# Bioinfo-Tools/PANGEA-plus

Hardware: AMD Instinct MI355X
Metric: classified reads/sec (+ HBM GB/s fraction), 150 bp vs 1 Gbp db, 1/2/4/8 GPU (higher is better)
Workload: dtype u64 (2-bit packed bases, integer scores)

## Files before the change

pangea-plus_amd/csrc/classify.hip:

```cpp
#include <algorithm>
#include <chrono>

#include "bitops.hpp"
#include "consensus_core.hpp"
#include "engine.hpp"

namespace pgx {

struct Diag {
	const uint64_t *rw, *ra;
	const uint64_t *dbw, *dba;
	int64_t dstart;
	int lo, hi;
};

template <bool AMB> __device__ __forceinline__ uint64_t mmw(const Diag &D, int w)
{
	int b0 = 32 * w;
	if (b0 + 32 <= D.lo || b0 >= D.hi)
		return kEven;
	uint64_t x = D.rw[w] ^ window64(D.dbw, D.dstart + b0);
	uint64_t m = (x | (x >> 1)) & kEven;
	if (AMB) {
		if (D.ra)
			m |= D.ra[w];
		if (D.dba)
			m |= window64(D.dba, D.dstart + b0);
	}
	m |= kEven & ~spaced_range(D.lo - b0, D.hi - b0);
	return m;
}

__device__ __forceinline__ uint64_t compress_even(uint64_t x)
{
	x = (x | (x >> 1)) & 0x3333333333333333ull;
	x = (x | (x >> 2)) & 0x0F0F0F0F0F0F0F0Full;
	x = (x | (x >> 4)) & 0x00FF00FF00FF00FFull;
	x = (x | (x >> 8)) & 0x0000FFFF0000FFFFull;
	x = (x | (x >> 16)) & 0x00000000FFFFFFFFull;
	return x;
}

template <bool AMB, int NW> struct DenseMask {
	static constexpr bool kHasWindows = true;
	static constexpr int kBits = 64 * NW;
	uint64_t m[NW];
	int lo, hi;
	__device__ __forceinline__ static uint64_t pick(const uint64_t (&a)[NW], int wi)
	{
		uint64_t v = 0;
#pragma unroll
		for (int k = 0; k < NW; k++)
			v = wi == k ? a[k] : v;
		return v;
	}
	__device__ __forceinline__ static uint64_t below(int n) { return n <= 0 ? 0ull : (n >= 64 ? ~0ull : ((1ull << n) - 1)); }
	__device__ __forceinline__ static uint64_t from(int n) { return n <= 0 ? ~0ull : (n >= 64 ? 0ull : (~0ull << n)); }
	__device__ __forceinline__ void build(const Diag &D)
	{
		lo = D.lo;
		hi = D.hi;
		const int64_t wi = D.dstart >> 5;
		const int sh = (int)(D.dstart & 31) * 2;
		uint64_t dbv[2 * NW + 1], rwv[2 * NW];
#pragma unroll
		for (int w = 0; w < 2 * NW + 1; w++)
			dbv[w] = D.dbw[wi + w];
#pragma unroll
		for (int w = 0; w < 2 * NW; w++)
			rwv[w] = D.rw[w];
		uint64_t d[2 * NW];
#pragma unroll
		for (int w = 0; w < 2 * NW; w++) {
			const uint64_t win = sh ? (dbv[w] >> sh) | (dbv[w + 1] << (64 - sh)) : dbv[w];
			const uint64_t x = rwv[w] ^ win;
			uint64_t mm = (x | (x >> 1)) & kEven;
			if (AMB) {
				if (D.ra)
					mm |= D.ra[w];
				if (D.dba)
					mm |= window64(D.dba, D.dstart + 32 * w);
			}
			d[w] = compress_even(mm);
		}
#pragma unroll
		for (int k = 0; k < NW; k++)
			m[k] = (d[2 * k] | (d[2 * k + 1] << 32)) | below(lo - 64 * k) | from(hi - 64 * k);
	}
	struct Win {
		uint64_t w[NW];
	};
	template <int K> __device__ __forceinline__ static void and_shr(const uint64_t (&a)[NW], const uint64_t (&src)[NW], uint64_t (&o)[NW])
	{
#pragma unroll
		for (int k = 0; k < NW; k++) {
			const uint64_t up = k + 1 < NW ? src[k + 1] : 0ull;
			o[k] = a[k] & ((src[k] >> K) | (up << (64 - K)));
		}
	}
	__device__ __forceinline__ Win seed_windows() const
	{
		uint64_t r[NW], a2[NW], a4[NW], a8[NW], b16[NW], c24[NW];
#pragma unroll
		for (int k = 0; k < NW; k++)
			r[k] = ~m[k];
		and_shr<1>(r, r, a2);
		and_shr<2>(a2, a2, a4);
		and_shr<4>(a4, a4, a8);
		and_shr<8>(a8, a8, b16);
		and_shr<16>(b16, a8, c24);
		Win w;
		and_shr<24>(c24, a4, w.w);
		return w;
	}
	__device__ __forceinline__ static bool win_any_below(const Win &w, int n)
	{
		uint64_t any = 0;
#pragma unroll
		for (int k = 0; k < NW; k++)
			any |= w.w[k] & below(n - 64 * k);
		return any != 0;
	}
	__device__ __forceinline__ static int first_set_ge(const uint64_t (&a)[NW], int n)
	{
		int r = kBits;
#pragma unroll
		for (int k = NW - 1; k >= 0; k--) {
			const uint64_t v = a[k] & from(n - 64 * k);
			r = v ? 64 * k + __ffsll((unsigned long long)v) - 1 : r;
		}
		return r;
	}
	__device__ __forceinline__ static int win_first_ge(const Win &w, int n) { return first_set_ge(w.w, n); }
	__device__ __forceinline__ bool flagged(int p) const { return (pick(m, p >> 6) >> (p & 63)) & 1ull; }
	__device__ __forceinline__ int count_range(int a, int b) const
	{
		a = a > lo ? a : lo;
		b = b < hi ? b : hi;
		int c = 0;
#pragma unroll
		for (int k = 0; k < NW; k++)
			c += __popcll(m[k] & from(a - 64 * k) & below(b - 64 * k));
		return c;
	}
	__device__ __forceinline__ int first_ge(int pos) const
	{
		if (pos >= hi)
			return hi;
		const int r = first_set_ge(m, pos);
		return r < hi ? r : hi;
	}
	__device__ __forceinline__ int last_lt(int pos) const
	{
		if (pos <= lo)
			return lo - 1;
		int r = -1;
#pragma unroll
		for (int k = 0; k < NW; k++) {
			const uint64_t v = m[k] & below(pos - 64 * k);
			r = v ? 64 * k + 63 - __clzll((long long)v) : r;
		}
		return r >= lo ? r : lo - 1;
	}
	struct Fwd {
		uint64_t w;
		int wi;
	};
	__device__ __forceinline__ Fwd fwd_from(int k) const
	{
		const int pos = k + 1;
		Fwd c;
		c.wi = pos >> 6;
		c.w = pick(m, c.wi) & (~0ull << (pos & 63));
		return c;
	}
	__device__ __forceinline__ int fwd_next(Fwd &c) const
	{
		while (!c.w) {
			c.wi++;
			if (c.wi >= NW)
				return hi;
			c.w = pick(m, c.wi);
		}
		const int r = c.wi * 64 + __ffsll((unsigned long long)c.w) - 1;
		c.w &= c.w - 1;
		return r < hi ? r : hi;
	}
	struct Bwd {
		uint64_t w;
		int wi;
	};
	__device__ __forceinline__ Bwd bwd_from(int k) const
	{
		Bwd c;
		if (k <= 0) {
			c.w = 0;
			c.wi = 0;
			return c;
		}
		const int q = k - 1, bb = q & 63;
		c.wi = q >> 6;
		c.w = pick(m, c.wi) & (bb == 63 ? ~0ull : ((2ull << bb) - 1));
		return c;
	}
	__device__ __forceinline__ int bwd_next(Bwd &c) const
	{
		while (!c.w) {
			if (c.wi == 0)
				return lo - 1;
			c.wi--;
			c.w = pick(m, c.wi);
		}
		const int bb = 63 - __clzll((long long)c.w);
		c.w ^= 1ull << bb;
		const int r = c.wi * 64 + bb;
		return r >= lo ? r : lo - 1;
	}
};

template <bool AMB> struct LazyMask {
	static constexpr bool kHasWindows = false;
	struct Win {
	};
	Diag D;
	int lo, hi;
	__device__ __forceinline__ void build(const Diag &d)
	{
		D = d;
		lo = d.lo;
		hi = d.hi;
	}
	__device__ __forceinline__ int count_range(int, int) const { return 15; }
	__device__ __forceinline__ bool flagged(int p) const { return first_ge(p) == p; }
	__device__ __forceinline__ int first_ge(int pos) const
	{
		if (pos >= hi)
			return hi;
		int w = pos >> 5;
		uint64_t m = mmw<AMB>(D, w) & ~((1ull << (2 * (pos & 31))) - 1);
		while (!m) {
			w++;
			if (32 * w >= hi)
				return hi;
			m = mmw<AMB>(D, w);
		}
		int r = 32 * w + ((__ffsll((unsigned long long)m) - 1) >> 1);
		return r < hi ? r : hi;
	}
	__device__ __forceinline__ int last_lt(int pos) const
	{
		if (pos <= lo)
			return lo - 1;
		int q = pos - 1, w = q >> 5, bit = q & 31;
		uint64_t keep = bit == 31 ? ~0ull : ((1ull << (2 * bit + 2)) - 1);
		uint64_t m = mmw<AMB>(D, w) & keep;
		while (!m) {
			if (32 * w <= lo)
				return lo - 1;
			w--;
			m = mmw<AMB>(D, w);
		}
		int r = 32 * w + ((63 - __clzll((long long)m)) >> 1);
		return r >= lo ? r : lo - 1;
	}
	struct Fwd {
		int k;
	};
	__device__ __forceinline__ Fwd fwd_from(int k) const { return Fwd{ k }; }
	__device__ __forceinline__ int fwd_next(Fwd &c) const { return c.k = first_ge(c.k + 1); }
	struct Bwd {
		int k;
	};
	__device__ __forceinline__ Bwd bwd_from(int k) const { return Bwd{ k }; }
	__device__ __forceinline__ int bwd_next(Bwd &c) const { return c.k = last_lt(c.k); }
};

constexpr int kStage = 128;
constexpr int kDeal = 2;
constexpr int kQueue = 64 * (kDeal + 1);
constexpr int kWavesPerBlock = 4;

typedef uint32_t u32x4 __attribute__((ext_vector_type(4)));
union HitWords {
	pgx_hit h;
	u32x4 v[2];
};
__device__ __forceinline__ void store_hit_stream(pgx_hit *p, const pgx_hit &h)
{
	HitWords w;
	w.h = h;
	u32x4 *d = reinterpret_cast<u32x4 *>(p);
	__builtin_nontemporal_store(w.v[0], d);
	__builtin_nontemporal_store(w.v[1], d + 1);
}


constexpr int kDiagSlots = 128;
constexpr int kDiagProbes = 8;
constexpr uint32_t kNoDiag = 0xFFFFFFFFu;

struct WaveLds {
	union {
		pgx_hit hit[kStage];
		uint4 chit[2 * kStage];
	};
	uint32_t qp[kQueue], qmeta[kQueue], qsubj[kQueue], qs0[kQueue], qs1[kQueue];
	uint32_t diag[2][2][kDiagSlots / 2];
	uint64_t uwin[2][2][8];
	unsigned int n[2];
	unsigned int direct[2];
};

struct OutView {
	pgx_hit *main, *ovf;
	uint8_t *main_key, *ovf_key;
	uint8_t *main_reg;
	int reg_shift;
	unsigned long long main_cap, ovf_cap;
	unsigned long long *counters;
};
constexpr unsigned int kChunk = 2048;

__device__ __forceinline__ uint4 pack_hit(const pgx_hit &h)
{
	const uint32_t minus = h.sstart > h.send;
	return make_uint4((uint32_t)h.subject, (uint32_t)h.sstart, (uint32_t)h.qstart | ((uint32_t)h.qend << 16) | (minus << 31),
			  (uint32_t)h.score | ((uint32_t)h.mismatch << 16) | ((uint32_t)h.gapopen << 24));
}

__device__ __forceinline__ pgx_hit unpack_hit(const uint4 c, uint32_t read)
{
	pgx_hit h;
	h.read = (int32_t)read;
	h.subject = (int32_t)c.x;
	h.sstart = (int32_t)c.y;
	h.qstart = (int32_t)(c.z & 0xFFFFu);
	h.qend = (int32_t)((c.z >> 16) & 0x7FFFu);
	const int span = h.qend - h.qstart;
	h.send = (c.z >> 31) ? h.sstart - span : h.sstart + span;
	h.score = (int32_t)(c.w & 0xFFFFu);
	h.mismatch = (uint16_t)((c.w >> 16) & 0xFFu);
	h.gapopen = (uint16_t)(c.w >> 24);
	return h;
}

__device__ __forceinline__ uint4 pack_seed(const pgx_hit &h)
{
	const uint32_t sd = (uint32_t)h.send;
	return make_uint4((uint32_t)h.subject, (uint32_t)h.sstart, (uint32_t)h.qend | (((sd >> 1) & 0x7FFu) << 15) | (sd << 31),
			  (uint32_t)h.mismatch | ((uint32_t)h.gapopen << 4) | ((sd >> 12) << 8));
}

__device__ __forceinline__ pgx_hit unpack_seed(const uint4 c, uint32_t read, uint32_t woff, int L)
{
	pgx_hit h;
	h.read = (int32_t)read;
	h.subject = (int32_t)c.x;
	h.qstart = (int32_t)woff;
	h.qend = (int32_t)(c.z & 0x7FFFu);
	h.sstart = (int32_t)c.y;
	h.send = (int32_t)((c.z >> 31) | (((c.z >> 15) & 0x7FFu) << 1) | ((c.w >> 8) << 12));
	h.score = L;
	h.mismatch = (uint16_t)(c.w & 15u);
	h.gapopen = (uint16_t)((c.w >> 4) & 15u);
	return h;
}

__device__ __forceinline__ uint8_t seed_key(const pgx_hit &h) { return (uint8_t)((h.mismatch & 15u) | ((h.gapopen & 15u) << 4)); }

template <bool PACKED>
__device__ __forceinline__ void emit_hit(WaveLds *st, int rs, const OutView &ov, const pgx_hit &h, bool gapped)
{
	unsigned int slot = atomicAdd(&st->n[rs], 1u);
	if (slot < (unsigned)kStage) {
		if (PACKED)
			st->chit[rs * kStage + slot] = gapped ? pack_seed(h) : pack_hit(h);
		else
			st->hit[slot] = h;
	} else {
		atomicAdd(&st->direct[rs], 1u);
		unsigned long long g = atomicAdd(&ov.counters[4], 1ull);
		if (g < ov.ovf_cap) {
			ov.ovf[g] = h;
			if (gapped)
				ov.ovf_key[g] = seed_key(h);
		}
	}
}

__device__ __forceinline__ bool uwin_any(const uint64_t *uw, int a, int b)
{
	if (b < a)
		return false;
	for (int w = a >> 6; w <= (b >> 6); w++) {
		uint64_t v = uw[w];
		if (w == (a >> 6))
			v &= ~0ull << (a & 63);
		if (w == (b >> 6) && (b & 63) != 63)
			v &= (2ull << (b & 63)) - 1ull;
		if (v)
			return true;
	}
	return false;
}

template <bool AMB, class Mask, class Emit>
__device__ __forceinline__ void process_candidate(const DbView &db, const uint64_t *rw, const uint64_t *ra, const uint64_t *uw, int L,
						   uint32_t read, uint32_t woff, int strand, int qp, uint32_t p, bool tested, bool claimed, uint32_t s,
						   uint32_t s_start, uint32_t s_end, Emit &emit, unsigned long long &n_runs)
{
	if (p + (uint32_t)kSeedK > s_end)
		return;
	Diag D;
	D.rw = rw;
	D.ra = ra;
	D.dbw = db.words;
	D.dba = db.amb;

	D.dstart = (int64_t)p - qp;
	if (AMB && db.amb && db.amb_blk) {
		const int64_t a = D.dstart > 0 ? D.dstart : 0, b = D.dstart + L - 1;
		uint32_t any = 0;
		for (int64_t blk = a >> kBlkShift; blk <= (b >> kBlkShift); blk++)
			any |= (db.amb_blk[blk >> 5] >> (blk & 31)) & 1u;
		if (!any)
			D.dba = nullptr;
	}
	int64_t lo64 = (int64_t)s_start - D.dstart, hi64 = (int64_t)s_end - D.dstart;
	D.lo = lo64 > 0 ? (int)lo64 : 0;
	D.hi = hi64 < L ? (int)hi64 : L;
	Mask M;
	M.build(D);
	if (PGX_DBG_STOP(db) == 4) {
		n_runs += (unsigned long long)(M.first_ge(qp) & 1);
		return;
	}

	int pos, run_start = 0;
	typename Mask::Win W;
	bool whole = false;
	if constexpr (Mask::kHasWindows)
		whole = claimed;
	if (whole) {
		if constexpr (Mask::kHasWindows) {
			W = M.seed_windows();
			if (uw) {
#pragma unroll
				for (int k = 0; k < Mask::kBits / 64; k++)
					W.w[k] &= uw[k];
			}
			run_start = Mask::win_first_ge(W, 0);
		}
		if (run_start >= D.hi)
			return;
		if (uw)
			run_start = M.last_lt(run_start) + 1;
		n_runs++;
		if (PGX_DBG_STOP(db) == 5 || PGX_DBG_STOP(db) == 6)
			return;
	} else {
		const int lm = M.last_lt(qp);
		if (!tested && qp >= kProbeStride && lm < qp - kProbeStride)
			return;
		const int re = M.first_ge(qp);
		if (re < qp + kSeedK)
			return;
		run_start = lm + 1;
		if (re - run_start < kWord)
			return;
		if constexpr (Mask::kHasWindows) {
			W = M.seed_windows();
			if (uw) {
#pragma unroll
				for (int k = 0; k < Mask::kBits / 64; k++)
					W.w[k] &= uw[k];
				if (Mask::win_first_ge(W, run_start) > re - kWord)
					return;
			}
			n_runs++;
			if (PGX_DBG_STOP(db) == 5)
				return;
			if (Mask::win_any_below(W, run_start))
				return;
		} else {
			if (uw && !uwin_any(uw, run_start, re - kWord))
				return;
			n_runs++;
			if (PGX_DBG_STOP(db) == 5)
				return;
			pos = D.lo;
			while (pos < run_start) {
				int m1 = M.first_ge(pos);
				if (m1 - pos >= kWord && (!uw || uwin_any(uw, pos, m1 - kWord)))
					return;
				pos = m1 + 1;
			}
		}
		if (PGX_DBG_STOP(db) == 6)
			return;
	}
	int covered = D.lo;
	pos = run_start;
	while (pos < D.hi) {
		const int e = M.first_ge(pos);
		const int len = e - pos;
		bool seeds = len >= kWord && pos >= covered;
		if constexpr (!Mask::kHasWindows)
			seeds = seeds && (!uw || uwin_any(uw, pos, e - kWord));
		if (seeds) {
			int best = 0, cur = 0, bl = pos, nmm = 0, mm_best = 0;
			int k = pos - 1;
			typename Mask::Bwd cl = M.bwd_from(k);
			while (k >= D.lo) {
				cur -= 2;
				nmm++;
				if (best - cur > kXdrop)
					break;
				const int p2 = M.bwd_next(cl);
				cur += k - 1 - p2;
				const bool up = cur > best;
				best = up ? cur : best;
				bl = up ? p2 + 1 : bl;
				mm_best = up ? nmm : mm_best;
				k = p2;
			}
			int bestr = 0, br = e - 1, mmr_best = 0;
			cur = 0;
			nmm = 0;
			k = e;
			typename Mask::Fwd cr = M.fwd_from(k);
			while (k < D.hi) {
				cur -= 2;
				nmm++;
				if (bestr - cur > kXdrop)
					break;
				const int n2 = M.fwd_next(cr);
				cur += n2 - (k + 1);
				const bool up = cur > bestr;
				bestr = up ? cur : bestr;
				br = up ? n2 - 1 : br;
				mmr_best = up ? nmm : mmr_best;
				k = n2;
			}
			pgx_hit h;
			h.read = (int32_t)read;
			h.subject = (int32_t)s;
			h.score = len + best + bestr;
			h.mismatch = (uint16_t)(mm_best + mmr_best);
			h.gapopen = 0;
			const int64_t sl = D.dstart + bl - (int64_t)s_start + 1, sr = D.dstart + br - (int64_t)s_start + 1;
			if (!strand) {
				h.qstart = bl + 1;
				h.qend = br + 1;
				h.sstart = (int32_t)sl;
				h.send = (int32_t)sr;
			} else {
				h.qstart = L - br;
				h.qend = L - bl;
				h.sstart = (int32_t)sr;
				h.send = (int32_t)sl;
			}
			if (db.gapped) {
				int q = bl + (br - bl) / 2;
				while (M.flagged(q))
					q--;
				int anchor = M.last_lt(q) + 1;
				anchor = anchor > bl ? anchor : bl;
				int b0l = 0, b0r = 0, kl = 14, kr = 14;
				if constexpr (Mask::kHasWindows) {
					const int ml = M.count_range(bl, anchor), mr = (int)h.mismatch - ml;
					b0l = ml <= 18 ? 2 * (anchor - bl) - 6 * ml : 0;
					b0r = mr <= 18 ? 2 * (br + 1 - anchor) - 6 * mr : 0;
					b0l = b0l > 0 && b0l < 2047 ? b0l : 0;
					b0r = b0r > 0 && b0r < 2047 ? b0r : 0;
					kl = (2 * anchor - b0l) / 5;
					kr = (2 * (L - anchor) - b0r) / 5;
					kl = kl < 14 ? kl : 14;
					kr = kr < 14 ? kr : 14;
					if (L > db.deep_from) {
						kl = (ml + (bl > 0 ? 10 : 0)) / 3;
						kr = (mr + (br + 1 < L ? 10 : 0)) / 3;
						kl = kl < 14 ? kl : 14;
						kr = kr < 14 ? kr : 14;
					}
				}
				h.qstart = (int32_t)woff;
				h.qend = anchor;
				h.sstart = (int32_t)(uint32_t)(D.dstart + anchor);
				h.send = strand | (b0l << 1) | (b0r << 12);
				h.score = L;
				h.mismatch = (uint16_t)kl;
				h.gapopen = (uint16_t)kr;
			}
			if (PGX_DBG_STOP(db) != 7)
				emit(h);
			covered = br + 1;
		}
		if constexpr (Mask::kHasWindows) {
			pos = Mask::win_first_ge(W, covered > e ? covered : e + 1);
			if (uw && pos < D.hi)
				pos = M.last_lt(pos) + 1;
		} else
			pos = covered > e + 1 ? covered : e + 1;
	}
}

__device__ __forceinline__ void lds_fence()
{
	asm volatile("s_waitcnt lgkmcnt(0)" ::: "memory");
	__builtin_amdgcn_wave_barrier();
}

template <bool AMB, int NW, bool LISTED, bool DUST>
__global__ __launch_bounds__(64 * kWavesPerBlock, NW == 8 ? 3 : 4) void k_seed_extend(DbView db, ReadsView rd, OutView ov,
								      uint32_t *__restrict__ read_cnt,
								      uint32_t *__restrict__ read_start)
{
	constexpr bool DENSE = NW > 0;
	constexpr int RPW = DENSE ? 2 : 1;
	constexpr int LPR = 64 / RPW;
	constexpr unsigned int SLOT_CAP = kStage;
	__shared__ WaveLds s_lds[kWavesPerBlock];
	const int wave = threadIdx.x >> 6, lane = threadIdx.x & 63;
	const int my_rs = lane / LPR, my_li = lane % LPR;
	WaveLds *st = &s_lds[wave];
	unsigned long long n_probe = 0, n_post = 0, n_runs = 0, n_main = 0, n_surv = 0;
	unsigned long long chunk_base = 0;
	unsigned int chunk_used = kChunk;
	const unsigned long long lt_mask = lane ? (~0ull >> (64 - lane)) : 0ull;

	for (uint32_t rbase = (blockIdx.x * kWavesPerBlock + wave) * RPW; rbase < rd.n; rbase += gridDim.x * kWavesPerBlock * RPW) {
		const bool hasB = RPW == 2 && rbase + 1 < rd.n;
		const uint32_t rA = LISTED ? rd.list[rbase] : rbase, rB = LISTED ? (hasB ? rd.list[rbase + 1] : 0u) : rbase + 1;
		const int LA = (int)rd.len[rA], LB = hasB ? (int)rd.len[rB] : 0;
		const uint32_t wA = rd.woff[rA], wB = hasB ? rd.woff[rB] : 0u;
		const int L = my_rs ? LB : LA;
		const uint32_t w0 = my_rs ? wB : wA;
		const int nps = L >= kSeedK ? (L - kSeedK) / kProbeStride + 1 : 0;
		const int P = 2 * nps;
		const int PA = LA >= kSeedK ? 2 * ((LA - kSeedK) / kProbeStride + 1) : 0;
		const int PB = LB >= kSeedK ? 2 * ((LB - kSeedK) / kProbeStride + 1) : 0;
		const int Pmax = PA > PB ? PA : PB;
		unsigned int emitted[2] = { 0, 0 }, q_n = 0;
		bool frag[2] = { false, false };
		if (lane == 0) {
			st->n[0] = st->n[1] = 0;
			st->direct[0] = st->direct[1] = 0;
		}
		if (RPW == 2) {
#pragma unroll
			for (int k = 0; k < 2 * kDiagSlots / 64; k++)
				(&st->diag[0][0][0])[k * 64 + lane] = kNoDiag;
		}
		const bool dustA = DUST && rd.dustwin_f && rd.dust_any[rA] != 0, dustB = DUST && rd.dustwin_f && hasB && rd.dust_any[rB] != 0;
		if (DUST && DENSE && (dustA || dustB) && lane < 32) {
			const int us = lane >> 4, ustr = (lane >> 3) & 1, uk = lane & 7;
			const int uL = us ? LB : LA;
			uint64_t v = 0;
			if ((us ? dustB : dustA) && uk < (uL + 63) / 64)
				v = (ustr ? rd.dustwin_r : rd.dustwin_f)[(us ? wB : wA) + uk];
			st->uwin[us][ustr][uk] = v;
		}
		lds_fence();

		auto spill = [&](int rs) {
			unsigned int n = st->n[rs];
			if (n > SLOT_CAP)
				n = SLOT_CAP;
			unsigned long long base = 0;
			if (lane == 0)
				base = atomicAdd(&ov.counters[4], (unsigned long long)n);
			base = __shfl(base, 0);
			for (unsigned int i = lane; i < n; i += 64)
				if (base + i < ov.ovf_cap) {
					const pgx_hit hh = RPW == 2 ? (db.gapped ? unpack_seed(st->chit[rs * SLOT_CAP + i], rs ? rB : rA, rs ? wB : wA, rs ? LB : LA)
										  : unpack_hit(st->chit[rs * SLOT_CAP + i], rs ? rB : rA))
								     : st->hit[i];
					ov.ovf[base + i] = hh;
					if (db.gapped)
						ov.ovf_key[base + i] = seed_key(hh);
				}
			if (rs)
				emitted[1] += n, frag[1] = true;
			else
				emitted[0] += n, frag[0] = true;
			lds_fence();
			if (lane == 0)
				st->n[rs] = 0;
			lds_fence();
		};

		auto drain = [&](unsigned int cnt) {
			q_n -= cnt;
			if ((unsigned)lane < cnt && PGX_DBG_STOP(db) != 3) {
				const uint32_t p = st->qp[q_n + lane], meta = st->qmeta[q_n + lane];
				const uint32_t sj = st->qsubj[q_n + lane], s0 = st->qs0[q_n + lane], s1 = st->qs1[q_n + lane];
				const int strand = (int)(meta >> 31), rs = (int)((meta >> 29) & 1), qp = (int)(meta & 0x0FFFFFFFu);
				const bool tested = (meta >> 30) & 1, claimed = (meta >> 28) & 1;
				const uint32_t cw0 = rs ? wB : wA, cr = rs ? rB : rA;
				const int cL = rs ? LB : LA;
				const uint64_t *rw = (strand ? rd.rc : rd.fwd) + cw0;
				const uint64_t *ra = nullptr;
				if (AMB) {
					const uint64_t *a = strand ? rd.rc_amb : rd.fwd_amb;
					ra = a ? a + cw0 : nullptr;
				}
				const uint64_t *uw = nullptr;
				if (DUST && (rs ? dustB : dustA))
					uw = DENSE ? st->uwin[rs][strand] : (strand ? rd.dustwin_r : rd.dustwin_f) + cw0;
				auto emit = [&](const pgx_hit &hh) { emit_hit<RPW == 2>(st, rs, ov, hh, db.gapped != 0); };
				if (DENSE)
					process_candidate<AMB, DenseMask<AMB, (NW > 0 ? NW : 3)>>(db, rw, ra, uw, cL, cr, cw0, strand, qp, p, tested, claimed, sj, s0, s1, emit, n_runs);
				else
					process_candidate<AMB, LazyMask<AMB>>(db, rw, ra, uw, cL, cr, cw0, strand, qp, p, tested, claimed, sj, s0, s1, emit, n_runs);
			}
			lds_fence();
			if (st->n[0] > SLOT_CAP / 2)
				spill(0);
			if (RPW == 2 && st->n[1] > SLOT_CAP / 2)
				spill(1);
		};

		for (int pbase = 0; pbase < Pmax; pbase += LPR) {
			const int pid = pbase + my_li;
			uint32_t cnt = 0, lo = 0;
			int strand = 0, qpos = 0;
			uint32_t wl = 0, wr = 0;
			uint32_t flank_amb = 0;
			if (pid < P && (my_rs == 0 || hasB)) {
				strand = pid >= nps;
				qpos = (pid - strand * nps) * kProbeStride;
				const uint64_t *rw = (strand ? rd.rc : rd.fwd) + w0;
				wl = qpos >= kProbeStride ? window16(rw, qpos - kProbeStride) : 0u;
				wr = window16(rw, qpos + kSeedK);
				if (AMB) {
					const uint64_t *ra0 = strand ? rd.rc_amb : rd.fwd_amb;
					if (ra0) {
						if (qpos >= kProbeStride && (window64(ra0 + w0, qpos - kProbeStride) & ((1ull << 26) - 1)))
							flank_amb |= 1;
						if (window64(ra0 + w0, qpos + kSeedK) & ((1ull << 24) - 1))
							flank_amb |= 2;
					}
				}
				bool ok = true;
				if (AMB) {
					const uint64_t *ra = strand ? rd.rc_amb : rd.fwd_amb;
					if (ra && (uint32_t)window64(ra + w0, qpos))
						ok = false;
				}
				if (ok) {
					uint32_t b = seed_bucket(window16(rw, qpos), db.bits);
					lo = __builtin_nontemporal_load(&db.bucket_off[b]);
					cnt = __builtin_nontemporal_load(&db.bucket_off[(uint64_t)b + 1]) - lo;
				}
				n_probe++;
			}
			uint32_t incl = cnt;
#pragma unroll
			for (int d = 1; d < 64; d <<= 1) {
				uint32_t t = __shfl_up(incl, d);
				if (lane >= d)
					incl += t;
			}
			const uint32_t excl = incl - cnt;
			const uint32_t T = __shfl(incl, 63);
			const uint32_t pbase_idx = lo - excl;
			const uint32_t pmeta = (uint32_t)qpos | (flank_amb << 28) | ((uint32_t)strand << 31);
			n_post += cnt;
			if (PGX_DBG_STOP(db) == 1)
				continue;
			for (uint32_t it = 0; it < T; it += 64 * kDeal) {
				bool active[kDeal], tested[kDeal], keep[kDeal];
				uint32_t pidx[kDeal], p[kDeal], sj[kDeal], s0[kDeal], s1[kDeal];
				int o_strand[kDeal], o_qpos[kDeal], o_rs[kDeal];
				uint32_t o_wl[kDeal], o_wr[kDeal], o_famb[kDeal];
#pragma unroll
				for (int u = 0; u < kDeal; u++) {
					const uint32_t item = it + 64 * u + lane;
					active[u] = item < T;
					const uint32_t key = active[u] ? item : T - 1;
					int o = 0;
#pragma unroll
					for (int step = 32; step >= 1; step >>= 1) {
						int cand = o + step;
						uint32_t e = __shfl(excl, cand & 63);
						if (cand < 64 && e <= key)
							o = cand;
					}
					pidx[u] = __shfl(pbase_idx, o) + key;
					const uint32_t m = __shfl(pmeta, o);
					o_strand[u] = (int)(m >> 31);
					o_qpos[u] = (int)(m & 0x0FFFFFFFu);
					o_famb[u] = AMB ? (m >> 28) & 3u : 0u;
					o_rs[u] = o / LPR;
					o_wl[u] = __shfl(wl, o);
					o_wr[u] = __shfl(wr, o);
				}
				uint32_t raw[kDeal];
				uint2 ctx[kDeal];
#pragma unroll
				for (int u = 0; u < kDeal; u++) {
					raw[u] = 0u;
					ctx[u] = make_uint2(0u, 0u);
					if (active[u]) {
						const uint32_t *rp = reinterpret_cast<const uint32_t *>(db.post_ctx + pidx[u]);
						raw[u] = __builtin_nontemporal_load(rp);
						ctx[u] = make_uint2(__builtin_nontemporal_load(rp + 1), __builtin_nontemporal_load(rp + 2));
					}
				}
				uint32_t xl[kDeal], xr[kDeal];
				bool lknown[kDeal], rknown[kDeal];
#pragma unroll
				for (int u = 0; u < kDeal; u++) {
					p[u] = raw[u];
					keep[u] = active[u];
					tested[u] = false;
					xl[u] = xr[u] = 0;
					lknown[u] = rknown[u] = false;
					if (active[u]) {
						const bool db_clean = !AMB || !(ctx[u].x >> 31);
						const uint32_t fa = AMB ? o_famb[u] : 0u;
						lknown[u] = db_clean && !(fa & 1u) && o_qpos[u] >= kProbeStride;
						rknown[u] = db_clean && !(fa & 2u);
						if (lknown[u]) {
							tested[u] = !((ctx[u].x >> 30) & 1u);
							xl[u] = ctx[u].x ^ o_wl[u];
						}
						if (rknown[u])
							xr[u] = ctx[u].y ^ o_wr[u];
					}
				}
#pragma unroll
				for (int u = 0; u < kDeal; u++) {
					if (keep[u]) {
						const uint32_t ml = (xl[u] | (xl[u] >> 1)) & 0x01555555u;
						const uint32_t mr = (xr[u] | (xr[u] >> 1)) & 0x00555555u;
						int la = o_qpos[u] >= kProbeStride ? (lknown[u] ? (ml ? 12 - ((31 - __clz((int)ml)) >> 1) : kProbeStride) : kProbeStride) : 0;
						int ra = rknown[u] ? (mr ? (__ffs((int)mr) - 1) >> 1 : kWord - kSeedK) : kWord - kSeedK;
						if (tested[u] && la == kProbeStride)
							keep[u] = false;
						const int room = (o_rs[u] ? LB : LA) - o_qpos[u] - kSeedK;
						ra = ra < room ? ra : room;
						if (la + ra < kWord - kSeedK)
							keep[u] = false;
					}
				}
				if (PGX_DBG_STOP(db) == 8) {
					for (int u = 0; u < kDeal; u++)
						n_runs += keep[u];
					continue;
				}
				uint4 bi[kDeal];
#pragma unroll
				for (int u = 0; u < kDeal; u++)
					bi[u] = keep[u] ? db.blk_info[p[u] >> kBlkShift] : make_uint4(0u, 0u, 0u, 0u);
#pragma unroll
				for (int u = 0; u < kDeal; u++) {
					sj[u] = bi[u].x;
					s0[u] = bi[u].y;
					s1[u] = bi[u].z;
					if (keep[u] && s1[u] <= p[u]) {
						sj[u]++;
						s0[u] = s1[u];
						s1[u] = bi[u].w;
						while (s1[u] <= p[u]) {
							sj[u]++;
							s0[u] = s1[u];
							s1[u] = db.seq_off[sj[u] + 1];
// ... 1353 lines not shown
```

Baseline: 122.0 million.

## Unify left/right X-drop walks into one forward bit-reversed cursor loop

Replaces the separate backward and forward mismatch-cursor X-drop extensions in the bitmask class with a single forward walk over a virtual word array. The left side is bit-reversed and sentinel words mark the boundaries, so both directions use one ctz-based iterator without per-step bounds checks. For small NW the two sides are merged into one predicated loop to cut divergence. The mismatch count is now derived algebraically from the score rather than counted per step, and the anchor search uses a vectorized last-clear-bit scan. This lowers branch overhead and loop bookkeeping, at the cost of extra bitreverse work and a risk of subtle boundary or mismatch-count differences.

```diff
diff --git a/pangea-plus_amd/csrc/classify.hip b/pangea-plus_amd/csrc/classify.hip
--- a/pangea-plus_amd/csrc/classify.hip
+++ b/pangea-plus_amd/csrc/classify.hip
@@ -132,7 +132,6 @@
 		return r;
 	}
 	__device__ __forceinline__ static int win_first_ge(const Win &w, int n) { return first_set_ge(w.w, n); }
-	__device__ __forceinline__ bool flagged(int p) const { return (pick(m, p >> 6) >> (p & 63)) & 1ull; }
 	__device__ __forceinline__ int count_range(int a, int b) const
 	{
 		a = a > lo ? a : lo;
@@ -162,59 +161,101 @@
 		}
 		return r >= lo ? r : lo - 1;
 	}
-	struct Fwd {
+	__device__ __forceinline__ int last_clear_le(int q) const
+	{
+		int r = -1;
+#pragma unroll
+		for (int k = 0; k < NW; k++) {
+			const uint64_t v = ~m[k] & below(q + 1 - 64 * k);
+			r = v ? 64 * k + 63 - __clzll((long long)v) : r;
+		}
+		return r;
+	}
+	static constexpr int kRight = 64 * (NW + 1);
+	__device__ __forceinline__ uint64_t walk_word(int v) const
+	{
+		const bool left = v < NW;
+		uint64_t x = pick(m, left ? NW - 1 - v : v - NW - 1);
+		x = left ? __builtin_bitreverse64(x) : x;
+		return v == NW || v == 2 * NW + 1 ? ~0ull : x;
+	}
+	struct Cursor {
 		uint64_t w;
 		int wi;
 	};
-	__device__ __forceinline__ Fwd fwd_from(int k) const
-	{
-		const int pos = k + 1;
-		Fwd c;
-		c.wi = pos >> 6;
-		c.w = pick(m, c.wi) & (~0ull << (pos & 63));
+	__device__ __forceinline__ Cursor walk_from(int k) const
+	{
+		const int p = k + 1;
+		Cursor c;
+		c.wi = p >> 6;
+		c.w = walk_word(c.wi) & (~0ull << (p & 63));
 		return c;
 	}
-	__device__ __forceinline__ int fwd_next(Fwd &c) const
-	{
-		while (!c.w) {
-			c.wi++;
-			if (c.wi >= NW)
-				return hi;
-			c.w = pick(m, c.wi);
-		}
-		const int r = c.wi * 64 + __ffsll((unsigned long long)c.w) - 1;
+	__device__ __forceinline__ int walk_next(Cursor &c) const
+	{
+		while (!c.w)
+			c.w = walk_word(++c.wi);
+		const int r = c.wi * 64 + (int)__builtin_ctzll(c.w);
 		c.w &= c.w - 1;
-		return r < hi ? r : hi;
-	}
-	struct Bwd {
-		uint64_t w;
-		int wi;
-	};
-	__device__ __forceinline__ Bwd bwd_from(int k) const
-	{
-		Bwd c;
-		if (k <= 0) {
-			c.w = 0;
-			c.wi = 0;
-			return c;
-		}
-		const int q = k - 1, bb = q & 63;
-		c.wi = q >> 6;
-		c.w = pick(m, c.wi) & (bb == 63 ? ~0ull : ((2ull << bb) - 1));
-		return c;
-	}
-	__device__ __forceinline__ int bwd_next(Bwd &c) const
-	{
-		while (!c.w) {
-			if (c.wi == 0)
-				return lo - 1;
-			c.wi--;
-			c.w = pick(m, c.wi);
-		}
-		const int bb = 63 - __clzll((long long)c.w);
-		c.w ^= 1ull << bb;
-		const int r = c.wi * 64 + bb;
-		return r >= lo ? r : lo - 1;
+		return r;
+	}
+	__device__ __forceinline__ int walk_side(int k, int h, int &end) const
+	{
+		Cursor c = walk_from(k);
+		int cur = 0, best = 0;
+		while (k < h) {
+			cur -= 2;
+			if (best - cur > kXdrop)
+				break;
+			const int n2 = walk_next(c);
+			cur += n2 - k - 1;
+			const bool up = cur > best;
+			best = up ? cur : best;
+			end = up ? n2 - 1 : end;
+			k = n2;
+		}
+		return best;
+	}
+	__device__ __forceinline__ void walks(int pos, int e, int &bl, int &br, int &gain, int &mm) const
+	{
+		const int kL = kBits - pos, kR = kRight + e, hR = kRight + hi;
+		int best = 0, end = 0, bestL = 0, endL = 0;
+		if constexpr (NW >= 8) {
+			bestL = walk_side(kL, kBits - lo, endL);
+			best = walk_side(kR, hR, end);
+		} else {
+			const bool right_empty = e >= hi;
+			const Cursor cR = walk_from(kR);
+			int k = kL, h = kBits - lo;
+			Cursor c = walk_from(k);
+			int cur = 0;
+			bool left = true, live;
+			do {
+				cur -= 2;
+				const bool stop = k >= h || best - cur > kXdrop;
+				const bool turn = stop && left;
+				live = !stop || (left && !right_empty);
+				bestL = turn ? best : bestL;
+				endL = turn ? end : endL;
+				cur = turn ? -2 : cur;
+				best = turn ? 0 : best;
+				k = turn ? kR : k;
+				h = turn ? hR : h;
+				c.w = turn ? cR.w : c.w;
+				c.wi = turn ? cR.wi : c.wi;
+				left = left && !stop;
+				const int n2 = walk_next(c);
+				cur += n2 - k - 1;
+				const bool up = live && cur > best;
+				best = up ? cur : best;
+				end = up ? n2 - 1 : end;
+				k = n2;
+			} while (live);
+		}
+		bl = bestL > 0 ? kBits - 1 - endL : pos;
+		br = best > 0 ? end - kRight : e - 1;
+		gain = bestL + best;
+		mm = ((pos - bl - bestL) + (br + 1 - e - best)) / 3;
 	}
 };
 
@@ -263,16 +304,51 @@
 		int r = 32 * w + ((63 - __clzll((long long)m)) >> 1);
 		return r >= lo ? r : lo - 1;
 	}
-	struct Fwd {
-		int k;
-	};
-	__device__ __forceinline__ Fwd fwd_from(int k) const { return Fwd{ k }; }
-	__device__ __forceinline__ int fwd_next(Fwd &c) const { return c.k = first_ge(c.k + 1); }
-	struct Bwd {
-		int k;
-	};
-	__device__ __forceinline__ Bwd bwd_from(int k) const { return Bwd{ k }; }
-	__device__ __forceinline__ int bwd_next(Bwd &c) const { return c.k = last_lt(c.k); }
+	__device__ __forceinline__ int last_clear_le(int q) const
+	{
+		while (flagged(q))
+			q--;
+		return q;
+	}
+	__device__ __forceinline__ void walks(int pos, int e, int &bl, int &br, int &gain, int &mm) const
+	{
+		int best = 0, cur = 0, nmm = 0, mm_best = 0;
+		bl = pos;
+		int k = pos - 1;
+		while (k >= lo) {
+			cur -= 2;
+			nmm++;
+			if (best - cur > kXdrop)
+				break;
+			const int p2 = last_lt(k);
+			cur += k - 1 - p2;
+			const bool up = cur > best;
+			best = up ? cur : best;
+			bl = up ? p2 + 1 : bl;
+			mm_best = up ? nmm : mm_best;
+			k = p2;
+		}
+		int bestr = 0, mmr_best = 0;
+		br = e - 1;
+		cur = 0;
+		nmm = 0;
+		k = e;
+		while (k < hi) {
+			cur -= 2;
+			nmm++;
+			if (bestr - cur > kXdrop)
+				break;
+			const int n2 = first_ge(k + 1);
+			cur += n2 - (k + 1);
+			const bool up = cur > bestr;
+			bestr = up ? cur : bestr;
+			br = up ? n2 - 1 : br;
+			mmr_best = up ? nmm : mmr_best;
+			k = n2;
+		}
+		gain = best + bestr;
+		mm = mm_best + mmr_best;
+	}
 };
 
 constexpr int kStage = 128;
@@ -508,45 +584,13 @@
 		if constexpr (!Mask::kHasWindows)
 			seeds = seeds && (!uw || uwin_any(uw, pos, e - kWord));
 		if (seeds) {
-			int best = 0, cur = 0, bl = pos, nmm = 0, mm_best = 0;
-			int k = pos - 1;
-			typename Mask::Bwd cl = M.bwd_from(k);
-			while (k >= D.lo) {
-				cur -= 2;
-				nmm++;
-				if (best - cur > kXdrop)
-					break;
-				const int p2 = M.bwd_next(cl);
-				cur += k - 1 - p2;
-				const bool up = cur > best;
-				best = up ? cur : best;
-				bl = up ? p2 + 1 : bl;
-				mm_best = up ? nmm : mm_best;
-				k = p2;
-			}
-			int bestr = 0, br = e - 1, mmr_best = 0;
-			cur = 0;
-			nmm = 0;
-			k = e;
-			typename Mask::Fwd cr = M.fwd_from(k);
-			while (k < D.hi) {
-				cur -= 2;
-				nmm++;
-				if (bestr - cur > kXdrop)
-					break;
-				const int n2 = M.fwd_next(cr);
-				cur += n2 - (k + 1);
-				const bool up = cur > bestr;
-				bestr = up ? cur : bestr;
-				br = up ? n2 - 1 : br;
-				mmr_best = up ? nmm : mmr_best;
-				k = n2;
-			}
+			int bl, br, gain, mm;
+			M.walks(pos, e, bl, br, gain, mm);
 			pgx_hit h;
 			h.read = (int32_t)read;
 			h.subject = (int32_t)s;
-			h.score = len + best + bestr;
-			h.mismatch = (uint16_t)(mm_best + mmr_best);
+			h.score = len + gain;
+			h.mismatch = (uint16_t)mm;
 			h.gapopen = 0;
 			const int64_t sl = D.dstart + bl - (int64_t)s_start + 1, sr = D.dstart + br - (int64_t)s_start + 1;
 			if (!strand) {
@@ -561,9 +605,7 @@
 				h.send = (int32_t)sl;
 			}
 			if (db.gapped) {
-				int q = bl + (br - bl) / 2;
-				while (M.flagged(q))
-					q--;
+				const int q = M.last_clear_le(bl + (br - bl) / 2);
 				int anchor = M.last_lt(q) + 1;
 				anchor = anchor > bl ? anchor : bl;
 				int b0l = 0, b0r = 0, kl = 14, kr = 14;
```

Result: faster. 125.6 million (median of 6 runs) (+3.0%).
